# AcherStyx/SSD-Object-Detection

Hardware: AMD Instinct MI355X
Metric: images/sec SSD300 train step, batch 64 (higher is better)
Workload: dtype bf16; 1 GPU; BASELINE configs[2]: SSD300 full train step (anchor match+encode, image normalisation, conv fwd, loss, conv bwd, per-variable clip (64 variables) + Adam), per-GPU batch 64, 80 classes, synthetic COCO-shaped boxes; per_gpu_batch=64, global_batch=64, parallelism=single

## Files before the change

ssd-object-detection_amd/csrc/conv_wgrad.hip:

```cpp
#include <cstdint>
#include "common.h"
#include <hip/hip_bf16.h>

#include "conv_common.h"
namespace {

constexpr int WG_LD = 288;

__device__ __forceinline__ void conv_wgrad_block(const bf16_raw* __restrict__ x, const bf16_raw* __restrict__ dy,
                                                 float* __restrict__ slab_w, float* __restrict__ slab_b, const ConvGeom& g,
                                                 int m_per_split, char* smem, const int bidx, const int bidy, const int bidz) {
    constexpr int TILE = 64 * WG_LD;
    auto s_dy = [&](int buf) { return smem + buf * (2 * TILE); };
    auto s_x = [&](int buf) { return smem + buf * (2 * TILE) + TILE; };

    const int tid = threadIdx.x, lane = tid & 63, wave = tid >> 6;
    const int wave_m = wave & 1, wave_n = wave >> 1;
    const int col0 = bidx * 128, co0 = bidy * 128;
    const int ktot = g.ldw;
    const int m_begin = bidz * m_per_split;
    const int m_end = min(g.M, m_begin + m_per_split);

    const int cslot = tid & 15, prow = tid >> 4;
    const int qx = (col0 >> 3) + cslot;
    const bool xcol_ok = qx < g.nchunks;
    const int tapx = xcol_ok ? qx / g.cpt : 0;
    const int ccx = qx - tapx * g.cpt;
    const int khx = tapx / g.KW, kwx = tapx - khx * g.KW;
    const int co_chunk = co0 + cslot * 8;
    const bool dycol_ok = co_chunk < g.N;

    uint4 rdy[4], rxx[4];
    auto load_tiles = [&](int mstep) {
#pragma unroll
        for (int j = 0; j < 4; ++j) {
            const int m = mstep + prow + 16 * j;
            const bool mok = m < m_end;
            rdy[j] = make_uint4(0, 0, 0, 0);
            rxx[j] = make_uint4(0, 0, 0, 0);
            if (mok && dycol_ok) rdy[j] = *reinterpret_cast<const uint4*>(dy + ((long long)m * g.N + co_chunk));
            if (mok && xcol_ok) {
                const int b = fdiv(m, g.d_hw);
                const int rem = m - b * g.d_hw.d;
                const int oy = fdiv(rem, g.d_w);
                const int ox = rem - oy * g.d_w.d;
                const int iy = oy * g.mul - g.pad_t + khx, ix = ox * g.mul - g.pad_l + kwx;
                if (iy >= 0 && iy < g.H && ix >= 0 && ix < g.W)
                    rxx[j] = *reinterpret_cast<const uint4*>(x + ((((long long)b * g.H + iy) * g.W + ix) * g.C + ccx * 8));
            }
        }
    };
    auto store_tiles = [&](int buf) {
#pragma unroll
        for (int j = 0; j < 4; ++j) {
            *reinterpret_cast<uint4*>(s_dy(buf) + (prow + 16 * j) * WG_LD + cslot * 16) = rdy[j];
            *reinterpret_cast<uint4*>(s_x(buf) + (prow + 16 * j) * WG_LD + cslot * 16) = rxx[j];
        }
    };

    f32x4_t acc[4][4];
    f32x4_t accb[4];
#pragma unroll
    for (int a = 0; a < 4; ++a) {
        accb[a] = f32x4_t{0.f, 0.f, 0.f, 0.f};
#pragma unroll
        for (int c = 0; c < 4; ++c) acc[a][c] = f32x4_t{0.f, 0.f, 0.f, 0.f};
    }
    const bool do_bias = slab_b != nullptr && bidx == 0 && wave_n == 0;
    bf16x8_t ones;
#pragma unroll
    for (int i = 0; i < 8; ++i) ones[i] = (__bf16)1.0f;

    const int nsteps = (m_end - m_begin + 63) / 64;
    if (nsteps > 0) {
        load_tiles(m_begin);
        store_tiles(0);
    }
    __syncthreads();
    const int gq = lane >> 4, li = lane & 15;
    const int tr_row = li >> 2, tr_col = (li & 3) * 4;
    for (int st = 0; st < nsteps; ++st) {
        const int cur = st & 1;
        const bool more = st + 1 < nsteps;
        if (more) load_tiles(m_begin + (st + 1) * 64);
#pragma unroll
        for (int ksub = 0; ksub < 2; ++ksub) {
            bf16x8_t fa[4], fb[4];
            const int krow = ksub * 32 + gq * 8 + tr_row;
#pragma unroll
            for (int a = 0; a < 4; ++a) {
                const char* base = s_dy(cur) + krow * WG_LD + (wave_m * 64 + a * 16 + tr_col) * 2;
                const s16x4_t lo = __builtin_amdgcn_ds_read_tr16_b64_v4i16((__attribute__((address_space(3))) s16x4_t*)(base));
                const s16x4_t hi = __builtin_amdgcn_ds_read_tr16_b64_v4i16((__attribute__((address_space(3))) s16x4_t*)(base + 4 * WG_LD));
                union { s16x4_t h[2]; bf16x8_t v; } u;
                u.h[0] = lo; u.h[1] = hi;
                fa[a] = u.v;
            }
#pragma unroll
            for (int c = 0; c < 4; ++c) {
                const char* base = s_x(cur) + krow * WG_LD + (wave_n * 64 + c * 16 + tr_col) * 2;
                const s16x4_t lo = __builtin_amdgcn_ds_read_tr16_b64_v4i16((__attribute__((address_space(3))) s16x4_t*)(base));
                const s16x4_t hi = __builtin_amdgcn_ds_read_tr16_b64_v4i16((__attribute__((address_space(3))) s16x4_t*)(base + 4 * WG_LD));
                union { s16x4_t h[2]; bf16x8_t v; } u;
                u.h[0] = lo; u.h[1] = hi;
                fb[c] = u.v;
            }
#pragma unroll
            for (int a = 0; a < 4; ++a)
#pragma unroll
                for (int c = 0; c < 4; ++c)
                    acc[a][c] = __builtin_amdgcn_mfma_f32_16x16x32_bf16(fa[a], fb[c], acc[a][c], 0, 0, 0);
            if (do_bias) {
#pragma unroll
                for (int a = 0; a < 4; ++a) accb[a] = __builtin_amdgcn_mfma_f32_16x16x32_bf16(fa[a], ones, accb[a], 0, 0, 0);
            }
        }
        if (more) store_tiles(cur ^ 1);
        __syncthreads();
    }
    float* out = slab_w + (long long)bidz * g.N * ktot;
#pragma unroll
    for (int a = 0; a < 4; ++a)
#pragma unroll
        for (int c = 0; c < 4; ++c) {
            const int col = col0 + wave_n * 64 + c * 16 + (lane & 15);
            if (col >= ktot) continue;
#pragma unroll
            for (int j = 0; j < 4; ++j) {
                const int co = co0 + wave_m * 64 + a * 16 + (lane >> 4) * 4 + j;
                if (co < g.N) out[(long long)co * ktot + col] = acc[a][c][j];
            }
        }
    if (do_bias && (lane & 15) == 0) {
        float* ob = slab_b + (long long)bidz * g.N;
#pragma unroll
        for (int a = 0; a < 4; ++a)
#pragma unroll
            for (int j = 0; j < 4; ++j) {
                const int co = co0 + wave_m * 64 + a * 16 + (lane >> 4) * 4 + j;
                if (co < g.N) ob[co] = accb[a][j];
            }
    }
}

__global__ __launch_bounds__(WG) void k_conv_wgrad(const bf16_raw* __restrict__ x, const bf16_raw* __restrict__ dy,
                                                   float* __restrict__ slab_w, float* __restrict__ slab_b, ConvGeom g,
                                                   int m_per_split) {
    extern __shared__ __attribute__((aligned(16))) char smem[];
    conv_wgrad_block(x, dy, slab_w, slab_b, g, m_per_split, smem, blockIdx.x, blockIdx.y, blockIdx.z);
}

constexpr int WGB_MAX = 8;
struct WgradBatchItem {
    const bf16_raw* x;
    const bf16_raw* dy;
    float* slab_w;
    float* slab_b;
    ConvGeom g;
    int mps, ctiles, mtiles, blk0;
};
struct WgradBatchArgs {
    int count;
    WgradBatchItem it[WGB_MAX];
};
__global__ __launch_bounds__(WG) void k_conv_wgrad_batched(WgradBatchArgs a) {
    extern __shared__ __attribute__((aligned(16))) char smem[];
    int l = 0;
#pragma unroll
    for (int k = 1; k < WGB_MAX; ++k) l += (k < a.count && (int)blockIdx.x >= a.it[k].blk0) ? 1 : 0;
    const WgradBatchItem& it = a.it[l];
    const int local = (int)blockIdx.x - it.blk0;
    const int per_split = it.ctiles * it.mtiles;
    const int bz = local / per_split, r = local - bz * per_split;
    const int by = r / it.ctiles, bx = r - by * it.ctiles;
    conv_wgrad_block(it.x, it.dy, it.slab_w, it.slab_b, it.g, it.mps, smem, bx, by, bz);
}

struct ReduceBatchItem {
    const float* slab_w;
    const float* slab_b;
    float* dw;
    float* db;
    long long sw, nw, sb;
    int nb, ns, blk0;
    unsigned nbw;
};
struct ReduceBatchArgs {
    int count;
    ReduceBatchItem it[WGB_MAX];
};
__global__ __launch_bounds__(256) void k_wgrad_reduce2_batched(ReduceBatchArgs a) {
    int l = 0;
#pragma unroll
    for (int k = 1; k < WGB_MAX; ++k) l += (k < a.count && (int)blockIdx.x >= a.it[k].blk0) ? 1 : 0;
    const ReduceBatchItem& it = a.it[l];
    const unsigned local = blockIdx.x - (unsigned)it.blk0;
    if (local < it.nbw) {
        const long long i = ((long long)local * 256 + threadIdx.x) * 4;
        if (i >= it.nw) return;
        float4 s = make_float4(0.f, 0.f, 0.f, 0.f);
        for (int z = 0; z < it.ns; ++z) {
            const float4 v = *reinterpret_cast<const float4*>(it.slab_w + (long long)z * it.sw + i);
            s.x += v.x; s.y += v.y; s.z += v.z; s.w += v.w;
        }
        *reinterpret_cast<float4*>(it.dw + i) = s;
    } else {
        const int i = (int)(local - it.nbw) * 256 + threadIdx.x;
        if (i >= it.nb) return;
        float s = 0.f;
        for (int z = 0; z < it.ns; ++z) s += it.slab_b[(long long)z * it.sb + i];
        it.db[i] = s;
    }
}


constexpr int WT_TILE = 64 * 512;
__global__ __launch_bounds__(512) void k_conv_wgrad_tile(const bf16_raw* __restrict__ x, const bf16_raw* __restrict__ dy,
                                                         float* __restrict__ slab_w, float* __restrict__ slab_b, ConvGeom g,
                                                         int m_per_split, int nsplit, int cout) {
    extern __shared__ __attribute__((aligned(16))) char smem[];
    const int tid = threadIdx.x, lane = tid & 63;
    const int wave = __builtin_amdgcn_readfirstlane(tid >> 6);
    const int wave_m = wave & 1, wave_n = wave >> 1;
    const int ktot = g.ldw;
    const int ctiles = (ktot + 255) >> 8, mtiles = (cout + 255) >> 8, tiles = ctiles * mtiles;
    int split, tile;
    if ((nsplit & 7) == 0) {
        const int kx = blockIdx.x >> 3;
        split = (kx / tiles) * 8 + (blockIdx.x & 7);
        tile = kx % tiles;
    } else {
        split = blockIdx.x / tiles;
        tile = blockIdx.x - split * tiles;
    }
    if (split >= nsplit) return;
    const int bx = tile % ctiles, by = tile / ctiles;
    const int col0 = bx * 256, co0 = by * 256;
    const int m_begin = split * m_per_split;
    const int m_end = min(g.M, m_begin + m_per_split);

    const __amdgpu_buffer_rsrc_t dyres = __builtin_amdgcn_make_buffer_rsrc((void*)dy, 0, (unsigned)g.M * (unsigned)g.N * 2u, 0x00020000);
    const __amdgpu_buffer_rsrc_t xres = __builtin_amdgcn_make_buffer_rsrc((void*)x, 0, (unsigned)g.B * g.H * g.W * g.C * 2u, 0x00020000);
    constexpr unsigned OOB = 0xfffffff0u;
    const int drow = lane >> 5;
    int rowj[4];
    unsigned dycol[4], xcol[4];
    int xkh[4], xkw[4];
#pragma unroll
    for (int j = 0; j < 4; ++j) {
        const int row = 2 * (wave + 8 * j) + drow;
        rowj[j] = row;
        const int pc = lane & 31;
        const int lg = ((pc >> 1) & 8) | (((pc >> 1) ^ row) & 7);
        const int ch = (lg * 2 + (pc & 1)) * 8;
        dycol[j] = co0 + ch < g.N ? (unsigned)(co0 + ch) * 2u : OOB;
        const int q = (col0 + ch) >> 3;
        if (q < g.nchunks) {
            const int tap = q / g.cpt;
            xcol[j] = (unsigned)(q - tap * g.cpt) * 16u;
            xkh[j] = tap / g.KW;
            xkw[j] = tap - xkh[j] * g.KW;
        } else {
            xcol[j] = OOB; xkh[j] = 0; xkw[j] = 0;
        }
    }
    const bool pointwise = g.KH == 1 && g.KW == 1 && g.mul == 1 && g.pad_t == 0 && g.pad_l == 0;
    constexpr int NJ = 2;
    constexpr int XOFF = WT_TILE / 2;
    auto issue_dma = [&](int mstep, int buf) {
        char* base = smem + buf * (2 * XOFF);
#pragma unroll
        for (int j = 0; j < NJ; ++j) {
            const int m = mstep + rowj[j];
            const bool mok = m < m_end;
            const unsigned od = (unsigned)m * (unsigned)g.N * 2u + dycol[j];
            __builtin_amdgcn_raw_ptr_buffer_load_lds(dyres, (lds_void*)(base + (wave + 8 * j) * 1024), 16,
                                                     (mok && dycol[j] != OOB) ? od : OOB, 0, 0, 0);
        }
#pragma unroll
        for (int j = 0; j < NJ; ++j) {
            const int m = mstep + rowj[j];
            bool ok = m < m_end && xcol[j] != OOB;
            unsigned pix;
            if (pointwise) {
                pix = (unsigned)m;
            } else {
                const int mm = ok ? m : 0;
                const int b = fdiv(mm, g.d_hw);
                const int rem = mm - b * g.d_hw.d;
                const int oy = fdiv(rem, g.d_w);
                const int ox = rem - oy * g.d_w.d;
                const int iy = oy * g.mul - g.pad_t + xkh[j], ix = ox * g.mul - g.pad_l + xkw[j];
                ok = ok && (unsigned)iy < (unsigned)g.H && (unsigned)ix < (unsigned)g.W;
                pix = (unsigned)((b * g.H + iy) * g.W + ix);
            }
            const unsigned ox_ = pix * (unsigned)g.C * 2u + xcol[j];
            __builtin_amdgcn_raw_ptr_buffer_load_lds(xres, (lds_void*)(base + XOFF + (wave + 8 * j) * 1024), 16,
                                                     ok ? ox_ : OOB, 0, 0, 0);
        }
    };

    f32x4_t acc[8][4];
    f32x4_t accb[8];
#pragma unroll
    for (int a = 0; a < 8; ++a) {
        accb[a] = f32x4_t{0.f, 0.f, 0.f, 0.f};
#pragma unroll
        for (int c = 0; c < 4; ++c) acc[a][c] = f32x4_t{0.f, 0.f, 0.f, 0.f};
    }
    const bool do_bias = slab_b != nullptr && bx == 0 && wave_n == 0;
    bf16x8_t ones;
#pragma unroll
    for (int i = 0; i < 8; ++i) ones[i] = (__bf16)1.0f;

    const int gq = lane >> 4, li = lane & 15;
    const int kk0 = (gq >> 1) * 16 + (gq & 1) * 4 + (li >> 2);
    const int key = kk0 & 7;
    int abase[8], bbase[4];
#pragma unroll
    for (int a = 0; a < 8; ++a) abase[a] = kk0 * 512 + ((wave_m * 8 + (a ^ key)) << 5) + (li & 3) * 8;
#pragma unroll
    for (int c = 0; c < 4; ++c) {
        const int gl = wave_n * 4 + c;
        bbase[c] = XOFF + kk0 * 512 + (((gl & 8) | ((gl & 7) ^ key)) << 5) + (li & 3) * 8;
    }
    auto rd = [&](int addr) { return lds_read_tr16_scoped(smem + addr, smem); };

    const int nsteps = (m_end - m_begin + 31) / 32;
#pragma unroll
    for (int p = 0; p < 3; ++p)
        if (p < nsteps) issue_dma(m_begin + p * 32, p);
    auto run = [&](auto bias_tag) {
        constexpr bool BIAS = decltype(bias_tag)::value;
        for (int st = 0; st < nsteps; ++st) {
            const int younger = min(2, nsteps - 1 - st);
            if (younger == 2) asm volatile("s_waitcnt vmcnt(8)" ::: "memory");
            else if (younger == 1) asm volatile("s_waitcnt vmcnt(4)" ::: "memory");
            else asm volatile("s_waitcnt vmcnt(0)" ::: "memory");
            __builtin_amdgcn_s_barrier();
            asm volatile("" ::: "memory");
            if (st + 3 < nsteps) issue_dma(m_begin + (st + 3) * 32, (st + 3) & 3);
            const int boff = (st & 3) * (2 * XOFF);
            bf16x8_t fb[4], fa[8];
#pragma unroll
            for (int c = 0; c < 4; ++c)
#pragma unroll
                for (int half = 0; half < 2; ++half)
                    reinterpret_cast<s16x4_t*>(&fb[c])[half] = rd(bbase[c] + boff + half * 4096);
#pragma unroll
            for (int a = 0; a < 8; ++a)
#pragma unroll
                for (int half = 0; half < 2; ++half)
                    reinterpret_cast<s16x4_t*>(&fa[a])[half] = rd(abase[a] + boff + half * 4096);
#pragma unroll
            for (int a = 0; a < 8; ++a) {
#pragma unroll
                for (int c = 0; c < 4; ++c)
                    acc[a][c] = __builtin_amdgcn_mfma_f32_16x16x32_bf16(fa[a], fb[c], acc[a][c], 0, 0, 0);
                if constexpr (BIAS) accb[a] = __builtin_amdgcn_mfma_f32_16x16x32_bf16(fa[a], ones, accb[a], 0, 0, 0);
            }
        }
    };
    if (do_bias) run(std::true_type{}); else run(std::false_type{});

    float* out = slab_w + (long long)split * g.N * ktot;
#pragma unroll
    for (int a = 0; a < 8; ++a)
#pragma unroll
        for (int c = 0; c < 4; ++c) {
            const int col = col0 + wave_n * 64 + c * 16 + (lane & 15);
            if (col >= ktot) continue;
#pragma unroll
            for (int j = 0; j < 4; ++j) {
                const int co = co0 + wave_m * 128 + a * 16 + (lane >> 4) * 4 + j;
                if (co < g.N) out[(long long)co * ktot + col] = acc[a][c][j];
            }
        }
    if (do_bias && (lane & 15) == 0) {
        float* ob = slab_b + (long long)split * g.N;
#pragma unroll
        for (int a = 0; a < 8; ++a)
#pragma unroll
            for (int j = 0; j < 4; ++j) {
                const int co = co0 + wave_m * 128 + a * 16 + (lane >> 4) * 4 + j;
                if (co < g.N) ob[co] = accb[a][j];
            }
    }
}

template <int BH, int BW8>
struct WpGeom {
    static constexpr int BW = BW8 * 8;
    static constexpr int PW = BW + 2, PH = BH + 2;
    static constexpr int PPIX = PW * PH;
    static constexpr int P_INSTR = (PPIX * 8 + 63) / 64;
    static constexpr int P_BYTES = P_INSTR * 1024;
    static constexpr int NPG = (BH / 2) * BW8;
    static constexpr int KS = (NPG + 1) / 2;
    static constexpr int DY_PIX = KS * 32;
    static constexpr int DY_BYTES = DY_PIX * 128;
    static constexpr int DY_INSTR = DY_PIX / 8;
    static constexpr int BUF = DY_BYTES + P_BYTES;
    static_assert(BH % 2 == 0 && DY_INSTR % 8 == 0, "block shape");
};

__device__ __forceinline__ int wp_key(int px) { return (px >> 1) & 3; }

template <int BH, int BW8>
__global__ __launch_bounds__(512) void k_conv3x3_wgrad_patch(const bf16_raw* __restrict__ x, const bf16_raw* __restrict__ dy,
                                                             float* __restrict__ slab_w, float* __restrict__ slab_b,
                                                             ConvGeom g, int tiles_x, int tiles_y, int tiles_per_split,
                                                             int nsplit, int cout, int single_buf, int xg) {
    using G = WpGeom<BH, BW8>;
    extern __shared__ __attribute__((aligned(16))) char smem[];

    const int tid = threadIdx.x, lane = tid & 63;
    const int wave = __builtin_amdgcn_readfirstlane(tid >> 6);
    const int ct = wave & 3, role = wave >> 2;
    const int nchunk = g.C >> 6, cotiles = (cout + 63) >> 6;
    const int nunits = nchunk * cotiles * nsplit;
    const int j = blockIdx.x >> 3;
    int id = ((j / xg) * 8 + (blockIdx.x & 7)) * xg + j % xg;
    if (id >= nunits) return;
    const int chunk = id % nchunk; id /= nchunk;
    const int cot = id % cotiles;
    const int split = id / cotiles;
    const int co0 = cot * 64, ci0 = chunk * 64;
    const int ntiles = g.B * tiles_x * tiles_y;
    const int t_begin = split * tiles_per_split, t_end = min(ntiles, t_begin + tiles_per_split);

    const __amdgpu_buffer_rsrc_t xres = __builtin_amdgcn_make_buffer_rsrc((void*)x, 0, (unsigned)g.B * g.H * g.W * g.C * 2u, 0x00020000);
    const __amdgpu_buffer_rsrc_t dyres = __builtin_amdgcn_make_buffer_rsrc((void*)dy, 0, (unsigned)g.B * g.Ho * g.Wo * g.N * 2u, 0x00020000);
    constexpr unsigned WP_OOB = 0xfffffff0u;
    auto issue_dma = [&](int t, int buf) {
        int r = t;
        const int tx = r % tiles_x; r /= tiles_x;
        const int ty = r % tiles_y;
        const int b = r / tiles_y;
        const int y0 = ty * BH, x0 = tx * G::BW;
        char* base = smem + buf * G::BUF;
#pragma unroll
        for (int j = 0; j < G::DY_INSTR / 4; ++j) {
            const int i = ct + 4 * j;
            const int kk = 8 * i + (lane >> 3), sl = lane & 7;
            const int c16 = (((sl >> 1) ^ wp_key(kk)) << 1) | (sl & 1);
            const int pg = kk >> 4;
            const int rp = pg / BW8, xg = pg - rp * BW8;
            const int y = y0 + 2 * rp + ((kk >> 3) & 1), xx = x0 + xg * 8 + (kk & 7);
            const int co = co0 + c16 * 8;
            const bool ok = pg < G::NPG && y < g.Ho && xx < g.Wo && co < g.N;
            const unsigned off = ((unsigned)((b * g.Ho + y) * g.Wo + xx) * (unsigned)g.N + (unsigned)co) * 2u;
            __builtin_amdgcn_raw_ptr_buffer_load_lds(dyres, (lds_void*)(base + i * 1024), 16, ok ? off : WP_OOB, 0, 0, 0);
        }
#pragma unroll
        for (int j = 0; j < (G::P_INSTR + 3) / 4; ++j) {
            const int i = ct + 4 * j;
            if (i < G::P_INSTR) {
                const int pp = 8 * i + (lane >> 3), sl = lane & 7;
                const int c16 = (((sl >> 1) ^ wp_key(pp)) << 1) | (sl & 1);
                const int py = pp / G::PW, px = pp - py * G::PW;
                const int iy = y0 - 1 + py, ix = x0 - 1 + px;
                const bool ok = pp < G::PPIX && (unsigned)iy < (unsigned)g.H && (unsigned)ix < (unsigned)g.W;
                const unsigned off = ((unsigned)((b * g.H + iy) * g.W + ix) * (unsigned)g.C + (unsigned)(ci0 + c16 * 8)) * 2u;
                __builtin_amdgcn_raw_ptr_buffer_load_lds(xres, (lds_void*)(base + G::DY_BYTES + i * 1024), 16, ok ? off : WP_OOB, 0, 0, 0);
            }
        }
    };

    constexpr int LTAPS = 4;
    f32x4_t acc[4][9 - LTAPS];
    f32x4_t accb[4];
#pragma unroll
    for (int a = 0; a < 4; ++a) {
        accb[a] = f32x4_t{0.f, 0.f, 0.f, 0.f};
#pragma unroll
        for (int t5 = 0; t5 < 9 - LTAPS; ++t5) acc[a][t5] = f32x4_t{0.f, 0.f, 0.f, 0.f};
    }
    const bool do_bias = slab_b != nullptr && chunk == 0 && ct == 0 && role == 1;
    bf16x8_t ones;
#pragma unroll
    for (int i = 0; i < 8; ++i) ones[i] = (__bf16)1.0f;

    if (t_begin < t_end && role == 0) issue_dma(t_begin, 0);
    const int gq = lane >> 4, li = lane & 15;
    int abase[4];
    {
        const int kk0 = (gq >> 1) * 8 + (gq & 1) * 4 + (li >> 2);
#pragma unroll
        for (int a = 0; a < 4; ++a) abase[a] = kk0 * 128 + ((a ^ wp_key(kk0)) << 5) + (li & 3) * 8;
    }
    int gbase[8];
    {
        const int p0 = (gq >> 1) * G::PW + (gq & 1) * 4 + (li >> 2);
#pragma unroll
        for (int r = 0; r < 8; ++r) gbase[r] = G::DY_BYTES + (p0 + r) * 128 + ((ct ^ wp_key(p0 + r)) << 5) + (li & 3) * 8;
    }
    typedef __attribute__((address_space(3))) s16x4_t lds_s16x4;
    struct Frag { bf16x8_t fa[4]; bf16x8_t fb[9 - LTAPS]; };
    auto run = [&](auto role_tag, auto bias_tag) {
        constexpr int ROLE = decltype(role_tag)::value;
        constexpr bool BIAS = decltype(bias_tag)::value;
        constexpr int TAP0 = ROLE == 0 ? 0 : LTAPS, NTAP = ROLE == 0 ? LTAPS : 9 - LTAPS;
        auto load_frag = [&](Frag& f, const int (&ab)[4], const int (&gb)[8], auto ks_tag) {
            constexpr int ks = decltype(ks_tag)::value;
#pragma unroll
            for (int half = 0; half < 2; ++half)
#pragma unroll
                for (int a = 0; a < 4; ++a)
                    reinterpret_cast<s16x4_t*>(&f.fa[a])[half] =
                        lds_read_tr16_scoped(smem + ab[a] + (ks * 2 + half) * 2048, smem);
#pragma unroll
            for (int t5 = 0; t5 < NTAP; ++t5)
#pragma unroll
                for (int half = 0; half < 2; ++half) {
                    const int tap = TAP0 + t5;
                    const int pg = (ks * 2 + half) < G::NPG ? (ks * 2 + half) : 0;
                    const int rp = pg / BW8, xg = pg - rp * BW8;
                    const int ctap = (2 * rp + tap / 3) * G::PW + xg * 8 + (tap % 3);
                    reinterpret_cast<s16x4_t*>(&f.fb[t5])[half] =
                        lds_read_tr16_scoped(smem + gb[ctap & 7] + (ctap >> 3) * 1024, smem);
                }
        };
        for (int t = t_begin; t < t_end; ++t) {
            const int cur = (t - t_begin) & 1;
            asm volatile("s_waitcnt vmcnt(0)" ::: "memory");
            __syncthreads();
            if constexpr (ROLE == 0) { if (t + 1 < t_end) issue_dma(t + 1, cur ^ 1); }
            const int boff = cur * G::BUF;
            int ab[4], gb[8];
#pragma unroll
            for (int a = 0; a < 4; ++a) ab[a] = abase[a] + boff;
#pragma unroll
            for (int r = 0; r < 8; ++r) gb[r] = gbase[r] + boff;
            Frag f0, f1;
            auto mma = [&](const Frag& f) {
#pragma unroll
                for (int t5 = 0; t5 < NTAP; ++t5)
#pragma unroll
                    for (int a = 0; a < 4; ++a)
                        acc[a][t5] = __builtin_amdgcn_mfma_f32_16x16x32_bf16(f.fa[a], f.fb[t5], acc[a][t5], 0, 0, 0);
                if constexpr (BIAS) {
#pragma unroll
                    for (int a = 0; a < 4; ++a) accb[a] = __builtin_amdgcn_mfma_f32_16x16x32_bf16(f.fa[a], ones, accb[a], 0, 0, 0);
                }
            };
            auto weave = [&]() {
                constexpr int NR = 8 + 2 * NTAP, NM = 4 * NTAP;
                constexpr int PAIRS = NR < NM ? NR : NM;
                if constexpr (NR > PAIRS) {
                    __builtin_amdgcn_sched_group_barrier(0x100, NR - PAIRS, 0);
                }
#pragma unroll
                for (int i = 0; i < PAIRS; ++i) {
                    __builtin_amdgcn_sched_group_barrier(0x008, 1, 0);
                    __builtin_amdgcn_sched_group_barrier(0x100, 1, 0);
                }
                constexpr int REST = NM - PAIRS + (BIAS ? 4 : 0);
                if constexpr (REST > 0) __builtin_amdgcn_sched_group_barrier(0x008, REST, 0);
            };
            static_assert(G::KS == 8, "the hand-unrolled pipeline below assumes eight k-steps per block");
            load_frag(f0, ab, gb, std::integral_constant<int, 0>{});
            __builtin_amdgcn_s_setprio(0);
            load_frag(f1, ab, gb, std::integral_constant<int, 1>{}); mma(f0); weave();
            load_frag(f0, ab, gb, std::integral_constant<int, 2>{}); mma(f1); weave();
            load_frag(f1, ab, gb, std::integral_constant<int, 3>{}); mma(f0); weave();
            load_frag(f0, ab, gb, std::integral_constant<int, 4>{}); mma(f1); weave();
            load_frag(f1, ab, gb, std::integral_constant<int, 5>{}); mma(f0); weave();
            load_frag(f0, ab, gb, std::integral_constant<int, 6>{}); mma(f1); weave();
            load_frag(f1, ab, gb, std::integral_constant<int, 7>{}); mma(f0); weave();
            mma(f1);
            __builtin_amdgcn_s_setprio(3);
        }
    };
    if (role == 0) run(std::integral_constant<int, 0>{}, std::false_type{});
    else if (do_bias) run(std::integral_constant<int, 1>{}, std::true_type{});
    else run(std::integral_constant<int, 1>{}, std::false_type{});
    const int ktot = g.ldw;
    float* out = slab_w + (long long)split * g.N * ktot;
    const int tap0 = role == 0 ? 0 : LTAPS, ntap = role == 0 ? LTAPS : 9 - LTAPS;
#pragma unroll
    for (int a = 0; a < 4; ++a)
#pragma unroll
        for (int t5 = 0; t5 < 9 - LTAPS; ++t5) {
            if (t5 >= ntap) continue;
            const int col = (tap0 + t5) * g.C + ci0 + ct * 16 + (lane & 15);
#pragma unroll
            for (int j = 0; j < 4; ++j) {
                const int co = co0 + a * 16 + (lane >> 4) * 4 + j;
                if (co < g.N) out[(long long)co * ktot + col] = acc[a][t5][j];
            }
        }
    if (do_bias && (lane & 15) == 0) {
        float* ob = slab_b + (long long)split * g.N;
#pragma unroll
        for (int a = 0; a < 4; ++a)
#pragma unroll
            for (int j = 0; j < 4; ++j) {
                const int co = co0 + a * 16 + (lane >> 4) * 4 + j;
                if (co < g.N) ob[co] = accb[a][j];
            }
    }
}

constexpr int W0_DY = 256 * 128;
constexpr int W0_PATCH = 6 * 1024;
constexpr int W0_BUF = W0_DY + W0_PATCH;

__global__ __launch_bounds__(512) void k_conv0_wgrad(const bf16_raw* __restrict__ x, const bf16_raw* __restrict__ dy,
                                                     float* __restrict__ slab_w, float* __restrict__ slab_b, ConvGeom g,
                                                     int tiles_x, int tiles_y, int tiles_per_split, int cout) {
    extern __shared__ __attribute__((aligned(16))) char smem[];
    const int tid = threadIdx.x, lane = tid & 63;
    const int wave = __builtin_amdgcn_readfirstlane(tid >> 6);
    const int split = blockIdx.x;
    const int ntiles = g.B * tiles_x * tiles_y;
    const int t_begin = split * tiles_per_split, t_end = min(ntiles, t_begin + tiles_per_split);

    auto issue_dma = [&](int t, int buf) {
        int r = t;
        const int tx = r % tiles_x; r /= tiles_x;
        const int ty = r % tiles_y;
        const int b = r / tiles_y;
        const int y0 = ty * 16, x0 = tx * 16;
        char* base = smem + buf * W0_BUF;
#pragma unroll
        for (int j = 0; j < 4; ++j) {
            const int i = wave + 8 * j;
            const int kk = 8 * i + (lane >> 3), sl = lane & 7;
            const int c16 = (((sl >> 1) ^ wp_key(kk)) << 1) | (sl & 1);
            const int pg = kk >> 4;
            const int y = y0 + 2 * (pg >> 1) + ((kk >> 3) & 1), xx = x0 + (pg & 1) * 8 + (kk & 7);
            const int co = c16 * 8;
            const bool ok = y < g.Ho && xx < g.Wo && co < g.N;
            const bf16_raw* src = ok ? dy + ((unsigned)((b * g.Ho + y) * g.Wo + xx) * (unsigned)g.N + (unsigned)co)
                                     : reinterpret_cast<const bf16_raw*>(g_zero16);
            __builtin_amdgcn_global_load_lds((gbl_void*)src, (lds_void*)(base + i * 1024), 16, 0, 0);
        }
        if (wave < 6) {
            const int pp = wave * 64 + lane;
            const int py = pp / PATCH_W, px = pp - py * PATCH_W;
            const int iy = y0 - 1 + py, ix = x0 - 1 + px;
            const bool ok = pp < PATCH_PIX && (unsigned)iy < (unsigned)g.H && (unsigned)ix < (unsigned)g.W;
            const bf16_raw* src = ok ? x + (unsigned)((b * g.H + iy) * g.W + ix) * 8u : reinterpret_cast<const bf16_raw*>(g_zero16);
            __builtin_amdgcn_global_load_lds((gbl_void*)src, (lds_void*)(base + W0_DY + wave * 1024), 16, 0, 0);
        }
    };

    f32x4_t acc[4][5];
    f32x4_t accb[4];
#pragma unroll
    for (int a = 0; a < 4; ++a) {
        accb[a] = f32x4_t{0.f, 0.f, 0.f, 0.f};
#pragma unroll
        for (int c = 0; c < 5; ++c) acc[a][c] = f32x4_t{0.f, 0.f, 0.f, 0.f};
    }
    bf16x8_t ones;
#pragma unroll
    for (int i = 0; i < 8; ++i) ones[i] = (__bf16)1.0f;

    const int gq = lane >> 4, li = lane & 15;
    const int kk0 = (gq >> 1) * 8 + (gq & 1) * 4 + (li >> 2);
    int abase[4];
#pragma unroll
    for (int a = 0; a < 4; ++a) abase[a] = wave * 4096 + kk0 * 128 + ((a ^ wp_key(kk0)) << 5) + (li & 3) * 8;
    const int p0 = (2 * wave + (gq >> 1)) * PATCH_W + (gq & 1) * 4 + (li >> 2);
    int bbase[5];
#pragma unroll
    for (int t = 0; t < 5; ++t) {
        int tap = 2 * t + ((li >> 1) & 1);
        if (tap > 8) tap = 8;
        bbase[t] = W0_DY + (p0 + (tap / 3) * PATCH_W + tap % 3) * 16 + (li & 1) * 8;
    }
    typedef __attribute__((address_space(3))) s16x4_t lds_s16x4;
    auto rd = [&](int addr) { return lds_read_tr16_scoped(smem + addr, smem); };

    if (t_begin < t_end) issue_dma(t_begin, 0);
    for (int t = t_begin; t < t_end; ++t) {
        const int cur = (t - t_begin) & 1;
        asm volatile("s_waitcnt vmcnt(0)" ::: "memory");
        __syncthreads();
        if (t + 1 < t_end) issue_dma(t + 1, cur ^ 1);
        const int boff = cur * W0_BUF;
        bf16x8_t fa[4], fb[5];
#pragma unroll
        for (int half = 0; half < 2; ++half) {
#pragma unroll
            for (int a = 0; a < 4; ++a) reinterpret_cast<s16x4_t*>(&fa[a])[half] = rd(boff + abase[a] + half * 2048);
#pragma unroll
            for (int c = 0; c < 5; ++c) reinterpret_cast<s16x4_t*>(&fb[c])[half] = rd(boff + bbase[c] + half * 8 * 16);
        }
#pragma unroll
        for (int a = 0; a < 4; ++a) {
#pragma unroll
            for (int c = 0; c < 5; ++c) acc[a][c] = __builtin_amdgcn_mfma_f32_16x16x32_bf16(fa[a], fb[c], acc[a][c], 0, 0, 0);
            accb[a] = __builtin_amdgcn_mfma_f32_16x16x32_bf16(fa[a], ones, accb[a], 0, 0, 0);
        }
    }
    __syncthreads();
    float* red = reinterpret_cast<float*>(smem);
    for (int w = 0; w < 8; ++w) {
        if (wave == w) {
#pragma unroll
            for (int a = 0; a < 4; ++a) {
#pragma unroll
                for (int c = 0; c < 6; ++c) {
                    f32x4_t v;
                    if (c < 5) v = acc[a][c < 5 ? c : 0]; else v = accb[a];
                    f32x4_t* slot = reinterpret_cast<f32x4_t*>(red + ((a * 6 + c) * 64 + lane) * 4);
                    if (w > 0) { const f32x4_t o = *slot; v[0] += o[0]; v[1] += o[1]; v[2] += o[2]; v[3] += o[3]; }
                    *slot = v;
                }
            }
        }
        __syncthreads();
    }
    const int ktot = g.ldw;
    for (int idx = tid; idx < 24 * 64; idx += 512) {
        const int tile = idx >> 6, l = idx & 63;
        const int a = tile / 6, c = tile - a * 6;
        const f32x4_t v = *reinterpret_cast<const f32x4_t*>(red + idx * 4);
#pragma unroll
        for (int j = 0; j < 4; ++j) {
            const int co = a * 16 + (l >> 4) * 4 + j;
            if (co >= g.N) continue;
            if (c < 5) {
                const int col = c * 16 + (l & 15);
                if (col < ktot) slab_w[((long long)split * g.N + co) * ktot + col] = v[j];
            } else if (slab_b != nullptr && (l & 15) == 0) {
                slab_b[(long long)split * g.N + co] = v[j];
            }
        }
    }
}

__global__ __launch_bounds__(256) void k_wgrad_reduce2(const float* __restrict__ slab_w, long long sw, long long nw,
                                                       float* __restrict__ dw, const float* __restrict__ slab_b, long long sb,
                                                       int nb, float* __restrict__ db, int nsplit, unsigned nbw) {
    if (blockIdx.x < nbw) {
        const long long i = ((long long)blockIdx.x * 256 + threadIdx.x) * 4;
        if (i >= nw) return;
        float4 s = make_float4(0.f, 0.f, 0.f, 0.f);
        for (int z = 0; z < nsplit; ++z) {
            const float4 v = *reinterpret_cast<const float4*>(slab_w + (long long)z * sw + i);
            s.x += v.x; s.y += v.y; s.z += v.z; s.w += v.w;
        }
        *reinterpret_cast<float4*>(dw + i) = s;
    } else {
        const int i = (int)(blockIdx.x - nbw) * 256 + threadIdx.x;
        if (i >= nb) return;
        float s = 0.f;
        for (int z = 0; z < nsplit; ++z) s += slab_b[(long long)z * sb + i];
        db[i] = s;
    }
}

__global__ __launch_bounds__(256) void k_wgrad_reduce_wide(const float* __restrict__ slab_w, long long sw, long long nw,
                                                          float* __restrict__ dw, const float* __restrict__ slab_b, long long sb,
                                                          int nb, float* __restrict__ db, int nsplit, unsigned nbw) {
    __shared__ float4 part[256];
    const int o = threadIdx.x & 15, grp = threadIdx.x >> 4;
    float4 s4 = make_float4(0.f, 0.f, 0.f, 0.f);
    if (blockIdx.x < nbw) {
        const long long i = ((long long)blockIdx.x * 16 + o) * 4;
        if (i < nw)
            for (int z = grp; z < nsplit; z += 16) {
                const float4 v = *reinterpret_cast<const float4*>(slab_w + (long long)z * sw + i);
                s4.x += v.x; s4.y += v.y; s4.z += v.z; s4.w += v.w;
            }
        part[threadIdx.x] = s4;
        __syncthreads();
        if (grp == 0 && i < nw) {
            float4 t = part[o];
            for (int k = 1; k < 16; ++k) { const float4 v = part[k * 16 + o]; t.x += v.x; t.y += v.y; t.z += v.z; t.w += v.w; }
            *reinterpret_cast<float4*>(dw + i) = t;
        }
    } else {
        const int i = (int)(blockIdx.x - nbw) * 16 + o;
        float sacc = 0.f;
        if (i < nb)
            for (int z = grp; z < nsplit; z += 16) sacc += slab_b[(long long)z * sb + i];
        part[threadIdx.x].x = sacc;
        __syncthreads();
        if (grp == 0 && i < nb) {
            float t = part[o].x;
            for (int k = 1; k < 16; ++k) t += part[k * 16 + o].x;
            db[i] = t;
        }
    }
}


bool wgrad_same3x3(const ssd_wgrad_item& it) {
    return it.ksize == 3 && it.stride == 1 && it.pad_t == 1 && it.pad_l == 1 && it.H == it.Ho && it.W == it.Wo;
}

bool wgrad_first_channels(int Cin, int Cout, int ldy, int ksize) { return Cin == 8 && Cout <= 64 && ldy <= 64 && ksize == 3; }
bool wgrad_first_layer(const ssd_wgrad_item& it) {
    return ssd_knob("SSD_WGRAD_FIRST", 1) && wgrad_first_channels(it.Cin, it.Cout, it.ldy, it.ksize) && wgrad_same3x3(it) &&
           it.H >= 16 && it.W >= 16;
}

bool wgrad_use_patch(const ssd_wgrad_item& it) {
    const int mn = ssd_knob("SSD_WGRAD_PATCH", 16);
    return mn > 0 && wgrad_same3x3(it) && it.Cin % 64 == 0 && it.H >= mn && it.W >= mn;
}

bool wgrad_tile_channels(int Cout, long long ktot) { return Cout > 128 && ktot >= 256; }
bool wgrad_use_tile(long long M, int Cout, int ldy, long long ktot, long long x_elems) {
    return ssd_knob("SSD_WGRAD_TILE", 1) && wgrad_tile_channels(Cout, ktot) && M >= 2048 && M * ldy < (1ll << 31) - 16 &&
           x_elems < (1ll << 31) - 16;
}

int wgrad_patch_shape(int Ho, int Wo, int* bh, int* bw) {
    static const int shapes[3][3] = {{16, 16, 16}, {6, 40, 15}, {10, 24, 15}};
    int best = 0;
    double best_cost = 0;
    for (int i = 0; i < 3; ++i) {
        const double cost = (double)((Ho + shapes[i][0] - 1) / shapes[i][0]) * ((Wo + shapes[i][1] - 1) / shapes[i][1]);
        if (i == 0 || cost < best_cost) { best = i; best_cost = cost; }
    }
    const int forced = ssd_knob("SSD_WGRAD_PATCH_SHAPE", -1);
    if (forced >= 0 && forced < 3) best = forced;
    *bh = shapes[best][0]; *bw = shapes[best][1];
    return best;
}

int wgrad_patch_plan(int B, int Ho, int Wo, int Cin, int Cout, int* tiles_x, int* tiles_y, int* tps, int* ns) {
    int bh, bw;
    const int shape = wgrad_patch_shape(Ho, Wo, &bh, &bw);
    *tiles_x = (Wo + bw - 1) / bw; *tiles_y = (Ho + bh - 1) / bh;
    const int ntiles = B * *tiles_x * *tiles_y;
    const int groups = (Cin / 64) * ((Cout + 63) / 64);
    int want = 256 / groups;
    if (want < 1) want = 1;
    if (want > ntiles) want = ntiles;
    *tps = (ntiles + want - 1) / want;
    *ns = (ntiles + *tps - 1) / *tps;
    return shape;
}

constexpr int WG_BMO = 128, WG_BNC = 128;

int wgrad_splits(long long M, int tiles) {
    long long want = 768 / tiles;
    long long maxs = (M + 511) / 512;
    if (want > maxs) want = maxs;
    if (want < 1) want = 1;
    if (want > 512) want = 512;
    return (int)want;
}

int wgrad_tile_splits(long long M, int tiles, long long slab_elems) {
    int best = 1;
    double best_cost = 0;
    const long long maxs = M / 256 > 0 ? M / 256 : 1;
    for (int ns = 1; ns <= 64 && ns <= maxs; ++ns) {
        const long long rounds = ((long long)tiles * ns + 255) / 256;
        const long long steps = ((M + ns - 1) / ns + 63) / 64;
        const double cost = (double)rounds * steps * 2.2 + (double)ns * slab_elems * 8.0 / 4.0e6;
        if (ns == 1 || cost < best_cost) { best = ns; best_cost = cost; }
    }
    return best;
}

size_t slab_bytes(int ns, int ldy, long long ktot) { return (size_t)ns * ((size_t)ldy * ktot + ldy) * sizeof(float); }
float* slab_bias(float* slab_w, int ns, int ldy, long long ktot) { return slab_w + (size_t)ns * ldy * ktot; }

struct WgradPlan {
    int id;
    int ns;
    int per_split;
    int tx, ty;
    int ctiles, mtiles;
    int xg;
    unsigned grid;
    long long ktot;
    int word() const { return id | (ns >= 32 ? SSD_PLAN_F_REDUCE_WIDE : 0); }
};

int wgrad_plan(const ssd_wgrad_item& it, WgradPlan* p) {
    if (!geom_ok(it.B, it.H, it.W, it.Cin, it.Ho, it.Wo, it.Cout, it.ksize) || it.stride <= 0 || it.ldy < it.Cout || it.ldy % 8)
        return SSD_ERR_VALUE;
    *p = WgradPlan{};
    const long long M = (long long)it.B * it.Ho * it.Wo, x_elems = (long long)it.B * it.H * it.W * it.Cin;
    const long long ktot = p->ktot = (long long)it.ksize * it.ksize * it.Cin;
    if (wgrad_first_layer(it)) {
        p->id = SSD_PLAN_WG_FIRST;
        p->tx = (it.Wo + 15) / 16; p->ty = (it.Ho + 15) / 16;
        const int ntiles = it.B * p->tx * p->ty, want = ntiles < 512 ? ntiles : 512;
        p->per_split = (ntiles + want - 1) / want;
        p->ns = (ntiles + p->per_split - 1) / p->per_split;
        p->grid = (unsigned)p->ns;
    } else if (wgrad_use_patch(it) && x_elems * 2 < (1ll << 32) - 16 && M * it.ldy * 2 < (1ll << 32) - 16) {
        const int shape = wgrad_patch_plan(it.B, it.Ho, it.Wo, it.Cin, it.Cout, &p->tx, &p->ty, &p->per_split, &p->ns);
        p->id = shape == 1 ? SSD_PLAN_WG_PATCH_6x40 : (shape == 2 ? SSD_PLAN_WG_PATCH_10x24 : SSD_PLAN_WG_PATCH_16x16);
        const int groups = (it.Cin / 64) * ((it.Cout + 63) / 64), nunits = groups * p->ns;
        p->xg = 1;
        for (int d = groups; d >= 1; --d) {
            if (groups % d) continue;
            const int ngr = (nunits + d - 1) / d;
            const int load = ((ngr + 7) / 8) * d, fair = (nunits + 7) / 8;
            if (load * 100 <= fair * 107) { p->xg = d; break; }
        }
        if (!ssd_knob("SSD_WGRAD_PATCH_XCD", 1)) p->xg = 1;
        p->grid = (unsigned)(8 * p->xg * ((nunits + 8 * p->xg - 1) / (8 * p->xg)));
    } else {
        const bool tile = wgrad_use_tile(M, it.Cout, it.ldy, ktot, x_elems);
        const int bmo = tile ? 256 : WG_BMO, bnc = tile ? 256 : WG_BNC;
        p->id = tile ? SSD_PLAN_WG_TILE : SSD_PLAN_WG_GENERIC;
        p->ctiles = (int)((ktot + bnc - 1) / bnc); p->mtiles = (it.Cout + bmo - 1) / bmo;
        p->ns = tile ? wgrad_tile_splits(M, p->ctiles * p->mtiles, (long long)it.ldy * ktot) : wgrad_splits(M, p->ctiles * p->mtiles);
        p->per_split = ((int)((M + p->ns - 1) / p->ns) + 63) / 64 * 64;
        p->grid = (unsigned)(p->ctiles * p->mtiles * p->ns);
    }
    return SSD_OK;
}

ConvGeom wgrad_geom(const ssd_wgrad_item& it) {
    return make_geom(it.B, it.H, it.W, it.Cin, it.Ho, it.Wo, it.ldy, it.ksize, it.ksize, it.stride, 1, it.pad_t, it.pad_l);
}

}

void ssd_launch_wgrad_reduce(hipStream_t s, const float* slab_w, long long sw, long long nw, float* dw, const float* slab_b,
                             long long sb, int nb, float* db, int ns) {
    if (ns >= 32) {
        const unsigned nbw = (unsigned)((nw / 4 + 15) / 16), nbb = db ? (unsigned)((nb + 15) / 16) : 0u;
        hipLaunchKernelGGL(k_wgrad_reduce_wide, dim3(nbw + nbb), dim3(256), 0, s, slab_w, sw, nw, dw, slab_b, sb, nb, db, ns, nbw);
    } else {
        const unsigned nbw = (unsigned)((nw / 4 + 255) / 256), nbb = db ? (unsigned)((nb + 255) / 256) : 0u;
        hipLaunchKernelGGL(k_wgrad_reduce2, dim3(nbw + nbb), dim3(256), 0, s, slab_w, sw, nw, dw, slab_b, sb, nb, db, ns, nbw);
    }
}

extern "C" {

static size_t wgrad_ws_bytes(const ssd_wgrad_item& it) {
    return ssd_conv2d_bwd_weight_workspace_bytes(it.B, it.Ho, it.Wo, it.Cin, it.Cout, it.ldy, it.ksize);
}

size_t ssd_conv2d_bwd_weight_workspace_bytes(int B, int Ho, int Wo, int Cin, int Cout, int ldy, int ksize) {
    if (B <= 0 || Ho <= 0 || Wo <= 0 || Cin <= 0 || Cout <= 0 || ldy < Cout || ksize <= 0) return 0;
    const long long ktot = (long long)ksize * ksize * Cin, M = (long long)B * Ho * Wo;
    const int tiles = (int)(((ktot + WG_BNC - 1) / WG_BNC) * ((Cout + WG_BMO - 1) / WG_BMO));
    int ns = wgrad_splits(M, tiles);
    if (wgrad_first_channels(Cin, Cout, ldy, ksize) && ns < 512) ns = 512;
    if (wgrad_tile_channels(Cout, ktot)) {
        const int ns2 = wgrad_tile_splits(M, (int)(((ktot + 255) / 256) * ((Cout + 255) / 256)), (long long)ldy * ktot);
        if (ns2 > ns) ns = ns2;
    }
    ssd_wgrad_item same = {};
    same.B = B; same.H = same.Ho = Ho; same.W = same.Wo = Wo; same.Cin = Cin; same.ksize = ksize;
    same.stride = same.pad_t = same.pad_l = 1;
    if (wgrad_use_patch(same)) {
        int tx, ty, tps, nsp;
        wgrad_patch_plan(B, Ho, Wo, Cin, Cout, &tx, &ty, &tps, &nsp);
        if (nsp > ns) ns = nsp;
    }
    return slab_bytes(ns, ldy, ktot);
}

static int conv2d_bwd_weight_impl(const ssd_wgrad_item& it, void* ws, size_t ws_bytes, void* stream) {
    WgradPlan p;
    if (!it.x || !it.dy || !it.dw || wgrad_plan(it, &p) != SSD_OK) return SSD_ERR_VALUE;
    if (!ws || ws_bytes < wgrad_ws_bytes(it)) return SSD_ERR_WORKSPACE;
    const ConvGeom g = wgrad_geom(it);
    const bf16_raw* x = static_cast<const bf16_raw*>(it.x);
    const bf16_raw* dy = static_cast<const bf16_raw*>(it.dy);
    float* slab_w = static_cast<float*>(ws);
    float* slab_b = slab_bias(slab_w, p.ns, it.ldy, p.ktot);
    float* sb = it.dbias ? slab_b : nullptr;
    hipStream_t s = (hipStream_t)stream;
#define SSD_LAUNCH_WP(BH_, BW8_)                                                                                    \
    do {                                                                                                            \
        using G_ = WpGeom<BH_, BW8_>;                                                                               \
        auto kern_ = k_conv3x3_wgrad_patch<BH_, BW8_>;                                                              \
        static OnceLds set_; if (ensure_lds(set_, reinterpret_cast<const void*>(kern_), (int)(2 * G_::BUF)) != 0) return SSD_ERR_LAUNCH; \
        hipLaunchKernelGGL(kern_, dim3(p.grid), dim3(512), (size_t)2 * G_::BUF, s, x, dy, slab_w, sb, g, p.tx, p.ty, p.per_split, \
                           p.ns, it.Cout, 0, p.xg);                                                                 \
    } while (0)
    switch (p.id) {
        case SSD_PLAN_WG_FIRST: {
            static OnceLds set; if (ensure_lds(set, reinterpret_cast<const void*>(k_conv0_wgrad), (int)(2 * W0_BUF)) != 0) return SSD_ERR_LAUNCH;
            hipLaunchKernelGGL(k_conv0_wgrad, dim3(p.grid), dim3(512), 2 * W0_BUF, s, x, dy, slab_w, sb, g, p.tx, p.ty, p.per_split, it.Cout);
            break;
        }
        case SSD_PLAN_WG_PATCH_16x16: SSD_LAUNCH_WP(16, 2); break;
        case SSD_PLAN_WG_PATCH_6x40: SSD_LAUNCH_WP(6, 5); break;
        case SSD_PLAN_WG_PATCH_10x24: SSD_LAUNCH_WP(10, 3); break;
        case SSD_PLAN_WG_TILE: {
            static OnceLds set; if (ensure_lds(set, reinterpret_cast<const void*>(k_conv_wgrad_tile), (int)(4 * WT_TILE)) != 0) return SSD_ERR_LAUNCH;
            hipLaunchKernelGGL(k_conv_wgrad_tile, dim3(p.grid), dim3(512), 4 * WT_TILE, s, x, dy, slab_w, sb, g, p.per_split, p.ns, it.Cout);
            break;
        }
        default: {
            const size_t lds = 4 * 64 * WG_LD;
            static OnceLds set; if (ensure_lds(set, reinterpret_cast<const void*>(k_conv_wgrad), (int)lds) != 0) return SSD_ERR_LAUNCH;
            hipLaunchKernelGGL(k_conv_wgrad, dim3(p.ctiles, p.mtiles, p.ns), dim3(WG), lds, s, x, dy, slab_w, sb, g, p.per_split);
        }
    }
#undef SSD_LAUNCH_WP
    if (hipGetLastError() != hipSuccess) return SSD_ERR_LAUNCH;
    ssd_launch_wgrad_reduce(s, slab_w, (long long)it.ldy * p.ktot, (long long)it.Cout * p.ktot, it.dw, slab_b, (long long)it.ldy,
                            it.Cout, it.dbias, p.ns);
    return ssd_launch_status();
}

int ssd_conv2d_bwd_weight(const void* x, const void* dy, float* dw, float* dbias, int B, int H, int W, int Cin, int Cout,
                          int ldy, int ksize, int stride, int pad_t, int pad_l, int Ho, int Wo, void* ws, size_t ws_bytes,
                          void* stream) {
    const ssd_wgrad_item it = {x, dy, dw, dbias, B, H, W, Cin, Cout, ldy, ksize, stride, pad_t, pad_l, Ho, Wo};
    return conv2d_bwd_weight_impl(it, ws, ws_bytes, stream);
}

int ssd_conv2d_bwd_weight_plan(int B, int H, int W, int Cin, int Cout, int ldy, int ksize, int stride, int pad_t, int pad_l,
                               int Ho, int Wo) {
    const ssd_wgrad_item it = {nullptr, nullptr, nullptr, nullptr, B, H, W, Cin, Cout, ldy, ksize, stride, pad_t, pad_l, Ho, Wo};
    WgradPlan p;
    const int rc = wgrad_plan(it, &p);
    return rc != SSD_OK ? rc : p.word();
}

size_t ssd_conv2d_bwd_weight_batched_workspace_bytes(const ssd_wgrad_item* items, int count) {
    if (!items || count <= 0) return 0;
    size_t tot = 0;
    for (int i = 0; i < count; ++i) tot += ssd_align_up(wgrad_ws_bytes(items[i]), 256);
    return tot;
}

int ssd_conv2d_bwd_weight_batched(const ssd_wgrad_item* items, int count, void* ws, size_t ws_bytes, void* stream) {
    if (!items || count <= 0) return SSD_ERR_VALUE;
    if (count > WGB_MAX) return SSD_ERR_UNSUPPORTED;
    if (!ws || ws_bytes < ssd_conv2d_bwd_weight_batched_workspace_bytes(items, count)) return SSD_ERR_WORKSPACE;
    WgradBatchArgs wa;
    ReduceBatchArgs ra;
    wa.count = ra.count = count;
    char* ptr = static_cast<char*>(ws);
    int blk = 0, rblk = 0;
    for (int i = 0; i < count; ++i) {
        const ssd_wgrad_item& it = items[i];
        WgradPlan p;
        if (!it.x || !it.dy || !it.dw || wgrad_plan(it, &p) != SSD_OK) return SSD_ERR_VALUE;
        if (p.id != SSD_PLAN_WG_GENERIC || p.ns >= 32) return SSD_ERR_UNSUPPORTED;
        float* slab_w = reinterpret_cast<float*>(ptr);
        float* slab_b = slab_bias(slab_w, p.ns, it.ldy, p.ktot);
        ptr += ssd_align_up(wgrad_ws_bytes(it), 256);
        wa.it[i] = WgradBatchItem{static_cast<const bf16_raw*>(it.x), static_cast<const bf16_raw*>(it.dy), slab_w,
                                  it.dbias ? slab_b : nullptr, wgrad_geom(it), p.per_split, p.ctiles, p.mtiles, blk};
        blk += (int)p.grid;
        const long long nw = (long long)it.Cout * p.ktot;
        const unsigned nbw = (unsigned)((nw / 4 + 255) / 256), nbb = it.dbias ? (unsigned)((it.Cout + 255) / 256) : 0u;
        ra.it[i] = ReduceBatchItem{slab_w, slab_b, it.dw, it.dbias, (long long)it.ldy * p.ktot, nw, (long long)it.ldy, it.Cout, p.ns, rblk, nbw};
        rblk += (int)(nbw + nbb);
    }
    for (int i = count; i < WGB_MAX; ++i) { wa.it[i] = wa.it[0]; wa.it[i].blk0 = blk; ra.it[i] = ra.it[0]; ra.it[i].blk0 = rblk; }
    hipStream_t s = (hipStream_t)stream;
    const size_t lds = 4 * 64 * WG_LD;
    static OnceLds attr_set; if (ensure_lds(attr_set, reinterpret_cast<const void*>(k_conv_wgrad_batched), (int)lds) != 0) return SSD_ERR_LAUNCH;
    hipLaunchKernelGGL(k_conv_wgrad_batched, dim3(blk), dim3(WG), lds, s, wa);
    if (hipGetLastError() != hipSuccess) return SSD_ERR_LAUNCH;
    hipLaunchKernelGGL(k_wgrad_reduce2_batched, dim3(rblk), dim3(256), 0, s, ra);
    return ssd_launch_status();
}

}
```

Before: 7431 images/sec.

## Software-pipeline LDS fragment reads and interleave DMA with MFMA in tiled wgrad

Restructures the main loop of the tiled weight-gradient kernel so that the LDS transpose reads for the next step are issued while the current step's MFMAs run. Buffer-to-LDS DMA instructions are interleaved between the MFMA groups, and sched_group_barrier hints shape the instruction order. The bias-gradient MFMAs are now spread across all four wave_n groups instead of being done only by wave_n==0, which evens out per-wave work. The cost is more register pressure from double-buffered fragments, plus more complex waitcnt logic that depends on a fixed ring of 4 buffers.

```diff
diff --git a/ssd-object-detection_amd/csrc/conv_wgrad.hip b/ssd-object-detection_amd/csrc/conv_wgrad.hip
--- a/ssd-object-detection_amd/csrc/conv_wgrad.hip
+++ b/ssd-object-detection_amd/csrc/conv_wgrad.hip
@@ -215,6 +215,7 @@
 
 
 constexpr int WT_TILE = 64 * 512;
+constexpr int WT_NBUF = 4;
 __global__ __launch_bounds__(512) void k_conv_wgrad_tile(const bf16_raw* __restrict__ x, const bf16_raw* __restrict__ dy,
                                                          float* __restrict__ slab_w, float* __restrict__ slab_b, ConvGeom g,
                                                          int m_per_split, int nsplit, int cout) {
@@ -267,20 +268,15 @@
     const bool pointwise = g.KH == 1 && g.KW == 1 && g.mul == 1 && g.pad_t == 0 && g.pad_l == 0;
     constexpr int NJ = 2;
     constexpr int XOFF = WT_TILE / 2;
-    auto issue_dma = [&](int mstep, int buf) {
-        char* base = smem + buf * (2 * XOFF);
+    struct DmaOff { unsigned dy[NJ], x[NJ]; };
+    auto dma_offsets = [&](int mstep) {
+        DmaOff o;
 #pragma unroll
         for (int j = 0; j < NJ; ++j) {
             const int m = mstep + rowj[j];
             const bool mok = m < m_end;
-            const unsigned od = (unsigned)m * (unsigned)g.N * 2u + dycol[j];
-            __builtin_amdgcn_raw_ptr_buffer_load_lds(dyres, (lds_void*)(base + (wave + 8 * j) * 1024), 16,
-                                                     (mok && dycol[j] != OOB) ? od : OOB, 0, 0, 0);
-        }
-#pragma unroll
-        for (int j = 0; j < NJ; ++j) {
-            const int m = mstep + rowj[j];
-            bool ok = m < m_end && xcol[j] != OOB;
+            o.dy[j] = (mok && dycol[j] != OOB) ? (unsigned)m * (unsigned)g.N * 2u + dycol[j] : OOB;
+            bool ok = mok && xcol[j] != OOB;
             unsigned pix;
             if (pointwise) {
                 pix = (unsigned)m;
@@ -294,21 +290,25 @@
                 ok = ok && (unsigned)iy < (unsigned)g.H && (unsigned)ix < (unsigned)g.W;
                 pix = (unsigned)((b * g.H + iy) * g.W + ix);
             }
-            const unsigned ox_ = pix * (unsigned)g.C * 2u + xcol[j];
-            __builtin_amdgcn_raw_ptr_buffer_load_lds(xres, (lds_void*)(base + XOFF + (wave + 8 * j) * 1024), 16,
-                                                     ok ? ox_ : OOB, 0, 0, 0);
-        }
+            o.x[j] = ok ? pix * (unsigned)g.C * 2u + xcol[j] : OOB;
+        }
+        return o;
     };
+    auto dma_instr = [&](const DmaOff& o, int buf, int i) {
+        char* base = smem + buf * (2 * XOFF);
+        if (i < NJ) __builtin_amdgcn_raw_ptr_buffer_load_lds(dyres, (lds_void*)(base + (wave + 8 * i) * 1024), 16, o.dy[i], 0, 0, 0);
+        else __builtin_amdgcn_raw_ptr_buffer_load_lds(xres, (lds_void*)(base + XOFF + (wave + 8 * (i - NJ)) * 1024), 16, o.x[i - NJ], 0, 0, 0);
+    };
 
     f32x4_t acc[8][4];
-    f32x4_t accb[8];
+    f32x4_t accb[2];
 #pragma unroll
     for (int a = 0; a < 8; ++a) {
-        accb[a] = f32x4_t{0.f, 0.f, 0.f, 0.f};
 #pragma unroll
         for (int c = 0; c < 4; ++c) acc[a][c] = f32x4_t{0.f, 0.f, 0.f, 0.f};
     }
-    const bool do_bias = slab_b != nullptr && bx == 0 && wave_n == 0;
+    accb[0] = accb[1] = f32x4_t{0.f, 0.f, 0.f, 0.f};
+    const bool do_bias = slab_b != nullptr && bx == 0;
     bf16x8_t ones;
 #pragma unroll
     for (int i = 0; i < 8; ++i) ones[i] = (__bf16)1.0f;
@@ -326,42 +326,84 @@
     }
     auto rd = [&](int addr) { return lds_read_tr16_scoped(smem + addr, smem); };
 
-    const int nsteps = (m_end - m_begin + 31) / 32;
-#pragma unroll
-    for (int p = 0; p < 3; ++p)
-        if (p < nsteps) issue_dma(m_begin + p * 32, p);
-    auto run = [&](auto bias_tag) {
-        constexpr bool BIAS = decltype(bias_tag)::value;
-        for (int st = 0; st < nsteps; ++st) {
-            const int younger = min(2, nsteps - 1 - st);
-            if (younger == 2) asm volatile("s_waitcnt vmcnt(8)" ::: "memory");
-            else if (younger == 1) asm volatile("s_waitcnt vmcnt(4)" ::: "memory");
-            else asm volatile("s_waitcnt vmcnt(0)" ::: "memory");
+    const int nsteps = max(0, (m_end - m_begin + 31) / 32);
+    constexpr int NDB = 1, NIP = 8 - NDB;
+    struct Late { bf16x8_t fb[4], fa[NDB]; };
+    auto read_b = [&](bf16x8_t& f, int c, int off) {
+#pragma unroll
+        for (int half = 0; half < 2; ++half) reinterpret_cast<s16x4_t*>(&f)[half] = rd(bbase[c] + off + half * 4096);
+    };
+    auto read_a = [&](bf16x8_t& f, int a, int off) {
+#pragma unroll
+        for (int half = 0; half < 2; ++half) reinterpret_cast<s16x4_t*>(&f)[half] = rd(abase[a] + off + half * 4096);
+    };
+    auto run = [&](auto bias_tag, auto phase_tag) {
+        constexpr int BW = decltype(bias_tag)::value;
+        constexpr int DPH = decltype(phase_tag)::value ? 1 : 0;
+        bf16x8_t fa[NIP];
+        Late l0, l1;
+        auto step = [&](int st, int buf, Late& cur, Late& nxt) {
+            asm volatile("s_waitcnt vmcnt(%0)" ::"n"(2 * NJ * (WT_NBUF - 2)) : "memory");
+            asm volatile("s_waitcnt lgkmcnt(0)" ::: "memory");
             __builtin_amdgcn_s_barrier();
             asm volatile("" ::: "memory");
-            if (st + 3 < nsteps) issue_dma(m_begin + (st + 3) * 32, (st + 3) & 3);
-            const int boff = (st & 3) * (2 * XOFF);
-            bf16x8_t fb[4], fa[8];
-#pragma unroll
-            for (int c = 0; c < 4; ++c)
-#pragma unroll
-                for (int half = 0; half < 2; ++half)
-                    reinterpret_cast<s16x4_t*>(&fb[c])[half] = rd(bbase[c] + boff + half * 4096);
-#pragma unroll
-            for (int a = 0; a < 8; ++a)
-#pragma unroll
-                for (int half = 0; half < 2; ++half)
-                    reinterpret_cast<s16x4_t*>(&fa[a])[half] = rd(abase[a] + boff + half * 4096);
+            const DmaOff o = dma_offsets(m_begin + (st + WT_NBUF) * 32);
+            const int noff = (buf + 1 == WT_NBUF ? 0 : buf + 1) * (2 * XOFF);
 #pragma unroll
             for (int a = 0; a < 8; ++a) {
+                const bf16x8_t& f = a < NIP ? fa[a] : cur.fa[a - NIP];
 #pragma unroll
                 for (int c = 0; c < 4; ++c)
-                    acc[a][c] = __builtin_amdgcn_mfma_f32_16x16x32_bf16(fa[a], fb[c], acc[a][c], 0, 0, 0);
-                if constexpr (BIAS) accb[a] = __builtin_amdgcn_mfma_f32_16x16x32_bf16(fa[a], ones, accb[a], 0, 0, 0);
-            }
-        }
+                    acc[a][c] = __builtin_amdgcn_mfma_f32_16x16x32_bf16(f, cur.fb[c], acc[a][c], 0, 0, 0);
+                if (BW >= 0 && (a >> 1) == BW)
+                    accb[a & 1] = __builtin_amdgcn_mfma_f32_16x16x32_bf16(f, ones, accb[a & 1], 0, 0, 0);
+                if ((a & 1) == DPH) dma_instr(o, buf, a >> 1);
+                if (a < NIP) read_a(fa[a], a, noff);
+                if (a < NDB) read_a(nxt.fa[a], NIP + a, noff);
+                else if (a < NDB + 4) read_b(nxt.fb[a - NDB], a - NDB, noff);
+            }
+#pragma unroll
+            for (int a = 0; a < 8; ++a) {
+                const int nr = a == 0 ? 0 : (a - 1 < NIP ? 2 : 0) + (a - 1 < NDB + 4 ? 2 : 0);
+                const int nm = 4 + (BW >= 0 && (a >> 1) == BW ? 1 : 0);
+#pragma unroll
+                for (int i = 0; i < nm; ++i) {
+                    if (i < nr) __builtin_amdgcn_sched_group_barrier(0x100, 1, 0);
+                    __builtin_amdgcn_sched_group_barrier(0x008, 1, 0);
+                    if (i == nm - 1 && (a & 1) == DPH) __builtin_amdgcn_sched_group_barrier(0x010, 1, 0);
+                }
+            }
+        };
+#pragma unroll
+        for (int p = 0; p < WT_NBUF; ++p) {
+            const DmaOff o = dma_offsets(m_begin + p * 32);
+#pragma unroll
+            for (int i = 0; i < 2 * NJ; ++i) dma_instr(o, p, i);
+        }
+        asm volatile("s_waitcnt vmcnt(%0)" ::"n"(2 * NJ * (WT_NBUF - 1)) : "memory");
+        __builtin_amdgcn_s_barrier();
+        asm volatile("" ::: "memory");
+#pragma unroll
+        for (int c = 0; c < 4; ++c) read_b(l0.fb[c], c, 0);
+#pragma unroll
+        for (int a = 0; a < 8; ++a) read_a(a < NIP ? fa[a] : l0.fa[a - NIP], a, 0);
+        int st = 0, buf = 0;
+        auto up = [](int b) { return b + 1 == WT_NBUF ? 0 : b + 1; };
+        for (; st + 1 < nsteps; st += 2) {
+            step(st, buf, l0, l1);
+            step(st + 1, up(buf), l1, l0);
+            buf = up(up(buf));
+        }
+        if (st < nsteps) step(st, buf, l0, l1);
+        asm volatile("s_waitcnt vmcnt(0)" ::: "memory");
     };
-    if (do_bias) run(std::true_type{}); else run(std::false_type{});
+    if (nsteps > 0) {
+        if (!do_bias) { if (wave_n < 2) run(std::integral_constant<int, -1>{}, std::false_type{}); else run(std::integral_constant<int, -1>{}, std::true_type{}); }
+        else if (wave_n == 0) run(std::integral_constant<int, 0>{}, std::false_type{});
+        else if (wave_n == 1) run(std::integral_constant<int, 1>{}, std::false_type{});
+        else if (wave_n == 2) run(std::integral_constant<int, 2>{}, std::true_type{});
+        else run(std::integral_constant<int, 3>{}, std::true_type{});
+    }
 
     float* out = slab_w + (long long)split * g.N * ktot;
 #pragma unroll
@@ -379,11 +421,11 @@
     if (do_bias && (lane & 15) == 0) {
         float* ob = slab_b + (long long)split * g.N;
 #pragma unroll
-        for (int a = 0; a < 8; ++a)
+        for (int t = 0; t < 2; ++t)
 #pragma unroll
             for (int j = 0; j < 4; ++j) {
-                const int co = co0 + wave_m * 128 + a * 16 + (lane >> 4) * 4 + j;
-                if (co < g.N) ob[co] = accb[a][j];
+                const int co = co0 + wave_m * 128 + (2 * wave_n + t) * 16 + (lane >> 4) * 4 + j;
+                if (co < g.N) ob[co] = accb[t][j];
             }
     }
 }
@@ -989,8 +1031,8 @@
         case SSD_PLAN_WG_PATCH_6x40: SSD_LAUNCH_WP(6, 5); break;
         case SSD_PLAN_WG_PATCH_10x24: SSD_LAUNCH_WP(10, 3); break;
         case SSD_PLAN_WG_TILE: {
-            static OnceLds set; if (ensure_lds(set, reinterpret_cast<const void*>(k_conv_wgrad_tile), (int)(4 * WT_TILE)) != 0) return SSD_ERR_LAUNCH;
-            hipLaunchKernelGGL(k_conv_wgrad_tile, dim3(p.grid), dim3(512), 4 * WT_TILE, s, x, dy, slab_w, sb, g, p.per_split, p.ns, it.Cout);
+            static OnceLds set; if (ensure_lds(set, reinterpret_cast<const void*>(k_conv_wgrad_tile), (int)(WT_NBUF * WT_TILE)) != 0) return SSD_ERR_LAUNCH;
+            hipLaunchKernelGGL(k_conv_wgrad_tile, dim3(p.grid), dim3(512), WT_NBUF * WT_TILE, s, x, dy, slab_w, sb, g, p.per_split, p.ns, it.Cout);
             break;
         }
         default: {
```

Measured after the change: 7472 images/sec, median of 6. No clear change (+0.5%).
